# zama-ai/bounty-matrix-inversion

Hardware: AMD Instinct MI355X
Metric: PBS/sec per GPU + encrypted n x n inverse wall-clock (n=2,3,4) (higher is better)
Workload: dtype u64/f64

## Files before the change

bounty-matrix-inversion_amd/csrc/bmi_kernels_t64f.hip:

```cpp
#include <hip/hip_runtime.h>

#include "bmi_internal.hpp"
#include "fft_half_f64.hpp"
#include "fft_wave_f64.hpp"
#include "pair_sync.hpp"
#include "phase_prof.hpp"
#include "t64_common.hpp"
#include "t64_half_steps.hpp"

using t64::i64;
using t64::u64;
using namespace fftw;

namespace {

PH_ARRAY(g_phase_f)
using t64::f64_to_word;
using t64::mod_ab;
using t64::Scheme;
#ifndef BMI_T64F_CTS
#define BMI_T64F_CTS 4
#endif
constexpr int TF_CTS = BMI_T64F_CTS;
constexpr int TF_LDS_WORDS = TW_WORDS + 2 * TF_CTS * (SCRATCH_WORDS + N) + TF_CTS * BMI_AT_WORDS + 4 * TF_CTS;
static_assert(TF_LDS_WORDS <= BMI_LDS_WORDS_MAX, "TF_LDS_WORDS exceeds the 160 KB of LDS");
static_assert(SCRATCH_WORDS >= N, "a tile carries 512 complex partial sums to the partner");
static_assert(TF_CTS % 2 == 0, "both wavefronts of a pair must be in the same barrier group");

__global__ void __launch_bounds__(256) k_bsk_to_fft_t64(const u64 *__restrict__ std_polys, double *__restrict__ limb_polys,
                                                        const double *__restrict__ g_tw, uint32_t n_polys, int prec) {
    const int limbs = t64::limbs_of(prec);
    __shared__ double lds[TW_WORDS + 4 * SCRATCH_WORDS];
    for (int i = threadIdx.x; i < TW_WORDS; i += blockDim.x) lds[i] = g_tw[i];
    __syncthreads();
    const int wave = threadIdx.x >> 6, lane = threadIdx.x & 63;
    const uint32_t item = blockIdx.x * 4 + wave;
    if (item >= n_polys * (uint32_t)limbs) return;
    const uint32_t poly = item / limbs;
    const int j = (int)(item % limbs);
    double *scratch = lds + TW_WORDS + wave * SCRATCH_WORDS;
    double x[16];
    static_for<0, 16>([&](auto J) { x[J] = (double)t64::limb_of((i64)std_polys[(size_t)poly * N + lane + 64 * J], j, prec); });
    forward(x, lane, lds, scratch);
    double2 *dst = reinterpret_cast<double2 *>(limb_polys + (size_t)item * N);
    static_for<0, 8>([&](auto Cc) { dst[Cc * 64 + lane] = double2{x[Cc], x[Cc + 8]}; });
}

template <int L, int BG, bool STATS, bool GLWE>
__global__ void __launch_bounds__(128 * TF_CTS)
    k_blind_rotate_t64f(const u64 *__restrict__ small_cts, const uint32_t *__restrict__ lut_ids, const u64 *__restrict__ luts,
                        const double *__restrict__ bsk, const double *__restrict__ g_tw, u64 *__restrict__ out,
                        uint32_t count, uint32_t n, unsigned long long *__restrict__ stat) {
    constexpr int CTS = TF_CTS;
    constexpr int LIMBS = Scheme<48>::LIMBS, LB = Scheme<48>::BITS, PRE = Scheme<48>::PRE, AB = 64 - PRE;
    static_assert(2.0 * L * N * (double)(1ull << (BG - 1)) * (double)(1ull << (LB - 1)) <= 0x1p45, "limb sums must stay below 2^45");
    static_assert(LIMBS == 2 && L * BG < AB, "two limbs; the decomposed bits lie inside the key precision");
    extern __shared__ double lds[];
    double *tiles = lds + TW_WORDS;
    double *accs = tiles + 2 * CTS * SCRATCH_WORDS;
    double *at_base = accs + 2 * CTS * N;
    uint32_t *flags = reinterpret_cast<uint32_t *>(at_base + CTS * BMI_AT_WORDS);
    const int wave = threadIdx.x >> 6, lane = threadIdx.x & 63;
    const int ctl = wave >> 1, c = wave & 1;
    if (threadIdx.x < 4 * CTS) flags[threadIdx.x] = 0;
    for (int i = threadIdx.x; i < TW_WORDS; i += blockDim.x) lds[i] = g_tw[i];
    const uint32_t ct_raw = blockIdx.x * CTS + ctl;
    const bool live = ct_raw < count;
    const uint32_t ct = live ? ct_raw : count - 1;
    double *tile = tiles + wave * SCRATCH_WORDS;
    const double *ptile = tiles + (wave ^ 1) * SCRATCH_WORDS;
    double *accf = accs + wave * N;
    uint16_t *at = reinterpret_cast<uint16_t *>(at_base + ctl * BMI_AT_WORDS);
    uint32_t *f_pub = flags + wave, *f_pub_partner = flags + (wave ^ 1);
    uint32_t *f_ack = flags + 2 * CTS + wave, *f_ack_partner = flags + 2 * CTS + (wave ^ 1);
    const u64 *lwe = small_cts + (size_t)ct * (n + 1);
    t64::stage_lwe<LOG_N + 1>(at, lwe, n, lane + 64 * c, 128);
    __syncthreads();
    {
        const u64 *tv = luts + (size_t)(lut_ids[ct] & (BMI_LUT_CAP - 1)) * N;
        const uint32_t bt = at[n];
        static_for<0, 16>([&](auto J) {
            const uint32_t e = (lane + 64 * J + bt) & (2 * N - 1);
            const u64 v = tv[e & (N - 1)];
            const u64 w0 = c ? ((e & N) ? (u64)0 - v : v) : (u64)0;
            t64::set_acc<PRE>(accf[lane + 64 * J], w0);
        });
    }

    uint32_t hand = 0;
    double dev = 0.0;
    PH_DECL();
    double keep[16];
    static_for<0, 16>([&](auto J) { keep[J] = accf[lane + 64 * J]; });
    for (uint32_t i = 0; i < n; i++) {
        PH_MARK(7);
        barrier_if(threadIdx.x >= 64 * CTS);
        PH_MARK(0);
        const uint32_t a_t = at[i];
        const double *bsk_c = bsk + ((size_t)i * 4 * L + c * 2 * L) * LIMBS * N;
        __builtin_amdgcn_s_setprio(0);
        wave_sync();
        double r[16];
        {
            double vr[16], vs[16];
            static_for<0, 16>([&](auto J) {
                vr[J] = accf[((lane + 2 * N - a_t) + 64 * J) & (N - 1)];
                vs[J] = keep[J];
            });
            sched_fence();
            static_for<0, 16>([&](auto J) {
                const uint32_t e = ((lane + 2 * N - a_t) + 64 * J) & (2 * N - 1);
                const double d = mod_ab<AB>(((e & N) ? -vr[J] : vr[J]) - vs[J]);
                r[J] = t64::rounded_top_f64<L, BG, AB>(d);
            });
        }
        PH_MARK(1);
        double X[L][16];
        auto row_ptr = [&](int t) {
            const int j = t / (2 * L), q = t % (2 * L), lev = q % L, col = q < L ? (c ^ 1) : c;
            return reinterpret_cast<const double2 *>(bsk_c + ((size_t)(lev * 2 + col) * LIMBS + j) * N);
        };
        double2 kb[2][8];
        auto fetch = [&](double2 (&dst)[8], int t) { static_for<0, 8>([&](auto P) { dst[P] = row_ptr(t)[P * 64 + lane]; }); };
        ForwardTwiddles ftw;
        load_forward_twiddles(ftw, lane, lds);
        sched_fence();
        static_for<0, L>([&](auto LEV) {
            constexpr int lev = L - 1 - LEV;
            pin();
            static_for<0, 16>([&](auto J) {
                if constexpr (lev == 0) {
                    X[0][J] = r[J];
                } else {
                    const double rn = __builtin_floor(__builtin_fma(r[J], 1.0 / (double)(1ull << BG), 0.5));
                    X[lev][J] = __builtin_fma(-(double)(1ull << BG), rn, r[J]);
                    r[J] = rn;
                }
            });
            if constexpr (lev == 0) {
                fetch(kb[0], 0);
                pin();
            }
            forward(X[lev], lane, ftw, tile);
        });
        __builtin_amdgcn_s_setprio(1);
        PH_MARK(2);
        barrier_if(threadIdx.x < 64 * CTS);
        PH_MARK(0);
        double acc[16];
        static_for<0, LIMBS * 2 * L>([&](auto T) {
            constexpr int t = T, j = t / (2 * L), q = t % (2 * L), lev = q % L, cur = t & 1;
            if constexpr (q == 0) hand++;
            if constexpr (t + 1 < LIMBS * 2 * L && q != 2 * L - 1) fetch(kb[cur ^ 1], t + 1);
            sched_fence();
            static_for<0, 8>([&](auto P) {
                const double xr = X[lev][P], xi = X[lev][P + 8];
                if constexpr (lev == 0) {
                    acc[P] = __builtin_fma(xr, kb[cur][P].x, -(xi * kb[cur][P].y));
                    acc[P + 8] = __builtin_fma(xr, kb[cur][P].y, xi * kb[cur][P].x);
                } else {
                    acc[P] = __builtin_fma(xr, kb[cur][P].x, __builtin_fma(-xi, kb[cur][P].y, acc[P]));
                    acc[P + 8] = __builtin_fma(xr, kb[cur][P].y, __builtin_fma(xi, kb[cur][P].x, acc[P + 8]));
                }
            });
            if constexpr (q == L - 1) {
                wave_sync();
                static_for<0, 8>([&](auto P) {
                    reinterpret_cast<double2 *>(tile)[P * 64 + lane] = double2{acc[P], acc[P + 8]};
                });
                pair_post(f_pub, hand);
            }
            pin();
            if constexpr (q == 2 * L - 1) {
                PH_MARK(3);
                pair_wait(f_pub_partner, hand);
                PH_MARK(4);
                static_for<0, 8>([&](auto P) {
                    const double2 p = reinterpret_cast<const double2 *>(ptile)[P * 64 + lane];
                    acc[P] += p.x;
                    acc[P + 8] += p.y;
                });
                pin();
                pair_ack(f_ack, hand);
                pin();
                PH_MARK(5);
                inverse(acc, lane, lds, tile, [&]() {
                    pin();
                    pair_wait(f_ack_partner, hand);
                    pin();
                });
                PH_MARK(6);
                if constexpr (t + 1 < LIMBS * 2 * L) {
                    fetch(kb[cur ^ 1], t + 1);
                    pin();
                }
                static_for<0, 16>([&](auto J) {
                    double x = __builtin_rint(acc[J]);
                    if constexpr (STATS) dev = __builtin_fmax(dev, __builtin_fabs(acc[J] - x));
                    if constexpr (j > 0) {
                        constexpr double W = (double)(1ull << (AB - LB * j));
                        x = __builtin_fma(-W, __builtin_rint(x * (1.0 / W)), x);
                        keep[J] = mod_ab<AB>(__builtin_fma(x, (double)(1ull << (LB * j)), accf[lane + 64 * J]));
                        accf[lane + 64 * J] = keep[J];
                    } else {
                        accf[lane + 64 * J] += x;
                    }
                });
                pin();
            }
        });
    }

    PH_MARK(7);
    PH_STORE(g_phase_f, wave, lane);
    if constexpr (STATS) atomicMax(stat, (unsigned long long)__double_as_longlong(dev));
    if (!live) return;
    wave_sync();
    if constexpr (GLWE) {
        u64 *g = out + (size_t)ct * (2 * N) + c * N;
        static_for<0, 16>([&](auto J) { t64::store_glwe_word<PRE, AB>(g, accf, t64::ResidueSlot<N, 0>{}, lane + 64 * J); });
        return;
    }
    u64 *o = out + (size_t)ct * (N + 1);
    if (c == 0) {
        static_for<0, 16>([&](auto J) {
            const uint32_t m = lane + 64 * J;
            const u64 v = f64_to_word(accf[m]) << PRE;
            if (m == 0) o[0] = v;
            else o[N - m] = (u64)0 - v;
        });
    } else if (lane == 0) {
        o[N] = f64_to_word(accf[0]) << PRE;
    }
}

using namespace t64h;
constexpr int LF_LDS_WORDS = ffth::HT_WORDS + 2 * N + 2 * H_MAX_L * N + 2 * 2 * N + BMI_AT_WORDS;
static_assert(LF_LDS_WORDS <= BMI_LDS_WORDS_MAX, "LF_LDS_WORDS exceeds the 160 KB of LDS");

__global__ void __launch_bounds__(256) k_bsk_to_latf_t64(const u64 *__restrict__ std_polys, double *__restrict__ lat_polys,
                                                         const double *__restrict__ g_tw_h, uint32_t n_polys, int prec) {
    const int limbs = t64::limbs_of(prec);
    __shared__ double lds[ffth::HT_WORDS + 4 * H_HALF];
    for (int i = threadIdx.x; i < ffth::HT_WORDS; i += blockDim.x) lds[i] = g_tw_h[i];
    __syncthreads();
    const int wave = threadIdx.x >> 6, lane = threadIdx.x & 63;
    const int h = wave & 1;
    const uint32_t item = blockIdx.x * 2 + (wave >> 1);
    const bool ok = item < n_polys * (uint32_t)limbs;
    const uint32_t poly = ok ? item / limbs : 0;
    const int j = ok ? (int)(item % limbs) : 0;
    double2 *tile = reinterpret_cast<double2 *>(lds + ffth::HT_WORDS + wave * H_HALF);
    if (ok) {
        double re[4], im[4];
        static_for<0, 4>([&](auto R) {
            const uint32_t m = 2 * (lane + 64 * R) + h;
            re[R] = (double)t64::limb_of((i64)std_polys[(size_t)poly * N + m], j, prec);
            im[R] = (double)t64::limb_of((i64)std_polys[(size_t)poly * N + m + 512], j, prec);
        });
        ffth::C v[4];
        forward_half_of(h, re, im, v, lane, lds);
        static_for<0, 4>([&](auto R) { tile[R * 64 + lane] = double2{v[R].r, v[R].i}; });
    }
    __syncthreads();
    if (ok) {
        const double2 *te = reinterpret_cast<const double2 *>(lds + ffth::HT_WORDS + (wave & ~1) * H_HALF), *to = te + H_HALF / 2;
        double2 *o = reinterpret_cast<double2 *>(lat_polys + (size_t)item * N);
        static_for<0, 2>([&](auto Q2) {
            const int q = (h * 2 + Q2) * 64 + lane;
            const double2 e = te[q], od = to[q];
            o[2 * q] = double2{e.x + od.x, e.y + od.y};
            o[2 * q + 1] = double2{e.x - od.x, e.y - od.y};
        });
    }
}

template <int L, int BG, bool STATS, bool GLWE>
__global__ void __launch_bounds__(H_THREADS)
    k_blind_rotate_lat_t64f(const u64 *__restrict__ small_cts, const uint32_t *__restrict__ lut_ids, const u64 *__restrict__ luts,
                            const double *__restrict__ bsk_latf, const double *__restrict__ g_tw_h, u64 *__restrict__ out,
                            uint32_t count, uint32_t n, unsigned long long *__restrict__ stat) {
    constexpr int LIMBS = Scheme<48>::LIMBS, LB = Scheme<48>::BITS, PRE = Scheme<48>::PRE, AB = 64 - PRE;
    static_assert(2.0 * L * N * (double)(1ull << (BG - 1)) * (double)(1ull << (LB - 1)) <= 0x1p45, "limb sums must stay below 2^45");
    static_assert(LIMBS == 2 && L <= H_MAX_L && L * BG < AB, "two limbs, at most three levels");
    extern __shared__ double lds[];
    double *acc = lds + ffth::HT_WORDS;
    double2 *tiles = reinterpret_cast<double2 *>(lds + ffth::HT_WORDS + 2 * N);
    double2 *SD = tiles + H_MAX_L * N;
    uint16_t *at = reinterpret_cast<uint16_t *>(SD + 2 * N);
    const int tid = threadIdx.x, wave = tid >> 6, lane = tid & 63;
    for (int i = tid; i < ffth::HT_WORDS; i += H_THREADS) lds[i] = g_tw_h[i];
    const uint32_t ct = blockIdx.x;
    const u64 *lwe = small_cts + (size_t)ct * (n + 1);
    t64::stage_lwe<LOG_N + 1>(at, lwe, n, tid, H_THREADS);
    __syncthreads();
    {
        const u64 *tv = luts + (size_t)(lut_ids[ct] & (BMI_LUT_CAP - 1)) * N;
        const uint32_t bt = at[n];
        t64::load_test_poly<N, PRE>(acc, acc_slot, tv, bt, tid);
    }
    __syncthreads();
    const int mj = tid >> 9, mo = (tid >> 8) & 1, mq = tid & 255;
    uint32_t since_centred = 0;
    double dev = 0.0;

    for (uint32_t i = 0; i < n; i++) {
        const uint32_t a_t = at[i];
        if (a_t == 0) continue;
        const double *bi = bsk_latf + (size_t)i * 4 * L * LIMBS * N;
        double2 klo[2 * L], khi[2 * L];
        static_for<0, 2 * L>([&](auto R) {
            const double2 *row = reinterpret_cast<const double2 *>(bi + ((size_t)(R * 2 + mo) * LIMBS + mj) * N);
            klo[R] = row[2 * mq];
            khi[R] = row[2 * mq + 1];
        });
        if (wave < 4 * L) {
            const int c = wave / (2 * L), lev = (wave % (2 * L)) >> 1, h = wave & 1;
            const double *ac = acc + c * N;
            double x[8];
            double vr[8], vs[8];
            const uint32_t e0 = (2 * lane + h + 2 * N - a_t) & (2 * N - 1);
            const uint32_t t0 = e0 >> 1, pbase = (e0 & 1) * H_HALF;
            static_for<0, 8>([&](auto J) {
                const uint32_t t = t0 + 64 * (J & 3) + 256 * (J >> 2);
                vr[J] = ac[pbase + (t & (H_HALF - 1))];
                vs[J] = ac[h * H_HALF + lane + 64 * (J & 3) + 256 * (J >> 2)];
            });
            static_for<0, 8>([&](auto J) {
                const uint32_t t = t0 + 64 * (J & 3) + 256 * (J >> 2);
                const double dd = mod_ab<AB>(((t >> 9) & 1) ? -vr[J] - vs[J] : vr[J] - vs[J]);
                x[J] = t64::digit<L, BG, AB>(dd, lev);
            });
            const double re[4] = {x[0], x[1], x[2], x[3]}, im[4] = {x[4], x[5], x[6], x[7]};
            ffth::C v[4];
            forward_half_of(h, re, im, v, lane, lds);
            double2 *tile = tiles + (size_t)(wave >> 1) * H_HALF + h * (H_HALF / 2);
            static_for<0, 4>([&](auto R) { tile[R * 64 + lane] = double2{v[R].r, v[R].i}; });
        }
        __syncthreads();
        {
            ffth::C ylo{0.0, 0.0}, yhi{0.0, 0.0};
            static_for<0, 2 * L>([&](auto R) {
                const double2 e = tiles[(size_t)R * H_HALF + mq], od = tiles[(size_t)R * H_HALF + H_HALF / 2 + mq];
                mac_pair(ylo, yhi, e, od, klo[R], khi[R]);
            });
            const double2 w = reinterpret_cast<const double2 *>(lds + ffth::HT_W)[mq];
            sum_diff_store(SD + (size_t)(mj * 2 + mo) * H_HALF, mq, ylo, yhi, w);
        }
        __syncthreads();
        if (wave < 4 * LIMBS) {
            const int j = wave >> 2, o = (wave >> 1) & 1, h = wave & 1;
            const double2 *sd = SD + (size_t)(j * 2 + o) * H_HALF + h * (H_HALF / 2);
            ffth::C v[4];
            read_sums(v, sd, lane);
            double re[4], im[4];
            if (h) ffth::inverse_half<1>(v, re, im, lane, lds);
            else ffth::inverse_half<0>(v, re, im, lane, lds);
            double *ao = acc + o * N + h * H_HALF + lane;
            static_for<0, 4>([&](auto R) {
                atomicAdd(ao + 64 * R, t64::place_limb<AB, LB, STATS>(re[R], j, dev));
                atomicAdd(ao + 64 * R + 256, t64::place_limb<AB, LB, STATS>(im[R], j, dev));
            });
        }
        __syncthreads();
        if (++since_centred == H_RECENTRE) {
            since_centred = 0;
            recentre<AB, 2>(acc, tid);
            __syncthreads();
        }
    }
    if constexpr (STATS) atomicMax(stat, (unsigned long long)__double_as_longlong(dev));
    if constexpr (GLWE) t64::store_glwe<N, PRE, AB>(out + (size_t)ct * (2 * N), acc, acc_slot, tid);
    else t64::extract_sample<N, PRE, AB>(out + (size_t)ct * (N + 1), acc, acc_slot, tid);
}

}

PH_EXPORT(bmi_debug_phase_prof_t64f, g_phase_f)

namespace bmit {

bool shape_supported_fft(int prec, uint32_t levels, uint32_t base_log) {
    return prec == 48 && base_log == 10 && (levels == 3 || levels == 2);
}

int launch_bsk_to_fft(const u64 *std_polys, double *limb_polys, const double *g_tw_fft, uint32_t n_polys, int prec, hipStream_t s) {
    if (prec != 48) return (int)hipErrorInvalidValue;
    const uint32_t items = n_polys * (uint32_t)t64::limbs_of(prec);
    hipLaunchKernelGGL(k_bsk_to_fft_t64, dim3((items + 3) / 4), dim3(256), 0, s, std_polys, limb_polys, g_tw_fft, n_polys, prec);
    BMI_LAUNCH_CHECK();
    return 0;
}

int launch_bsk_to_latf(const u64 *std_polys, double *lat_polys, const double *g_tw_h, uint32_t n_polys, int prec, hipStream_t s) {
    if (prec != 48 && prec != 42) return (int)hipErrorInvalidValue;
    const uint32_t items = n_polys * (uint32_t)t64::limbs_of(prec);
    hipLaunchKernelGGL(k_bsk_to_latf_t64, dim3((items + 1) / 2), dim3(256), 0, s, std_polys, lat_polys, g_tw_h, n_polys, prec);
    BMI_LAUNCH_CHECK();
    return 0;
}

int launch_blind_rotate_lat_fft(const u64 *small_cts, const uint32_t *lut_ids, const u64 *luts, const double *bsk_fft,
                                const double *g_tw_fft, u64 *out, uint32_t count, uint32_t n, int prec, uint32_t levels,
                                uint32_t base_log, unsigned long long *stat, bool glwe, hipStream_t s) {
    if (count == 0) return 0;
    if (!shape_supported_fft(prec, levels, base_log)) return (int)hipErrorInvalidValue;
    return with_levels_stats_glwe(levels, stat != nullptr, glwe, [&](auto L, auto STATS, auto GLWE) {
        return launch_with_lds<k_blind_rotate_lat_t64f<L, 10, STATS, GLWE>>(dim3(count), dim3(H_THREADS), (size_t)LF_LDS_WORDS * sizeof(double), s,
                                                                             small_cts, lut_ids, luts, bsk_fft, g_tw_fft, out, count, n, stat);
    });
}

int launch_blind_rotate_fft(const u64 *small_cts, const uint32_t *lut_ids, const u64 *luts, const double *bsk_fft,
                            const double *g_tw_fft, u64 *out, uint32_t count, uint32_t n, int prec, uint32_t levels,
                            uint32_t base_log, unsigned long long *stat, bool glwe, hipStream_t s) {
    if (count == 0) return 0;
    if (!shape_supported_fft(prec, levels, base_log)) return (int)hipErrorInvalidValue;
    return with_levels_stats_glwe(levels, stat != nullptr, glwe, [&](auto L, auto STATS, auto GLWE) {
        return launch_with_lds<k_blind_rotate_t64f<L, 10, STATS, GLWE>>(dim3((count + TF_CTS - 1) / TF_CTS), dim3(128 * TF_CTS),
                                                                         (size_t)TF_LDS_WORDS * sizeof(double), s, small_cts, lut_ids, luts, bsk_fft,
                                                                         g_tw_fft, out, count, n, stat);
    });
}

}
```

bounty-matrix-inversion_amd/csrc/fft_wave_f64.hpp:

```cpp
#pragma once
#include <type_traits>

#include <hip/hip_runtime.h>

namespace fftw {

constexpr int LOG_N = 10;
constexpr int N = 1 << LOG_N;
constexpr int ROWC = 72;
constexpr int SCRATCH_WORDS = 8 * ROWC * 2;
constexpr int TW_T1 = 0;
constexpr int TW_T2 = 1024;
constexpr int TW_WORDS = 1024 + 128;

template <int I, int E, class F>
__device__ __forceinline__ void static_for(F &&f) {
    if constexpr (I < E) {
        f(std::integral_constant<int, I>{});
        static_for<I + 1, E>(f);
    }
}

__device__ __forceinline__ void wave_sync() {
    __builtin_amdgcn_fence(__ATOMIC_RELEASE, "wavefront");
    __builtin_amdgcn_wave_barrier();
    __builtin_amdgcn_fence(__ATOMIC_ACQUIRE, "wavefront");
}
__device__ __forceinline__ void sched_fence() { __builtin_amdgcn_sched_barrier(0); }

struct C {
    double r, i;
};
__device__ __forceinline__ C operator+(C a, C b) { return C{a.r + b.r, a.i + b.i}; }
__device__ __forceinline__ C operator-(C a, C b) { return C{a.r - b.r, a.i - b.i}; }
template <bool INV>
__device__ __forceinline__ C mul_i(C a) {
    if constexpr (INV) return C{a.i, -a.r};
    else return C{-a.i, a.r};
}
template <bool INV>
__device__ __forceinline__ C cmul(C a, double wr, double wi) {
    if constexpr (INV) return C{__builtin_fma(a.r, wr, a.i * wi), __builtin_fma(a.i, wr, -(a.r * wi))};
    else return C{__builtin_fma(a.r, wr, -(a.i * wi)), __builtin_fma(a.r, wi, a.i * wr)};
}
__device__ __forceinline__ C fma_h(C a, C b, double sh) { return C{__builtin_fma(sh, b.r, a.r), __builtin_fma(sh, b.i, a.i)}; }

__device__ constexpr double TWIST_C[8] = {1.0, 0.98078528040323043, 0.92387953251128674, 0.83146961230254524,
                                          0.70710678118654757, 0.55557023301960229, 0.38268343236508984, 0.19509032201612833};
__device__ constexpr double TWIST_S[8] = {0.0, 0.19509032201612825, 0.38268343236508978, 0.55557023301960218,
                                          0.70710678118654746, 0.83146961230254524, 0.92387953251128674, 0.98078528040323043};

template <bool INV>
__device__ __forceinline__ void dft8(C (&x)[8]) {
    constexpr double s = INV ? -1.0 : 1.0;
    constexpr double h = 0.70710678118654752440;
    const C a0 = x[0] + x[4], d0 = x[0] - x[4];
    const C a1 = x[1] + x[5], t1 = x[1] - x[5];
    const C a2 = x[2] + x[6], t2 = x[2] - x[6];
    const C a3 = x[3] + x[7], t3 = x[3] - x[7];
    const C d1 = C{t1.r - s * t1.i, t1.i + s * t1.r};
    const C d2 = mul_i<INV>(t2);
    const C d3 = C{-t3.r - s * t3.i, s * t3.r - t3.i};
    const C b0 = a0 + a2, b2 = a0 - a2;
    const C b1 = a1 + a3, b3 = mul_i<INV>(a1 - a3);
    const C e0 = d0 + d2, e2 = d0 - d2;
    const C e1 = d1 + d3, e3 = mul_i<INV>(d1 - d3);
    x[0] = b0 + b1;
    x[4] = b0 - b1;
    x[2] = b2 + b3;
    x[6] = b2 - b3;
    x[1] = fma_h(e0, e1, h);
    x[5] = fma_h(e0, e1, -h);
    x[3] = fma_h(e2, e3, h);
    x[7] = fma_h(e2, e3, -h);
}

struct NoHook {
    __device__ __forceinline__ void operator()() const {}
};

template <bool INV, class Pre, class Emit>
__device__ __forceinline__ void dft8_emit(C (&x)[8], Pre &&pre, Emit &&emit) {
    constexpr double s = INV ? -1.0 : 1.0;
    constexpr double h = 0.70710678118654752440;
    const C a0 = x[0] + x[4], d0 = x[0] - x[4];
    const C a1 = x[1] + x[5], t1 = x[1] - x[5];
    const C a2 = x[2] + x[6], t2 = x[2] - x[6];
    const C a3 = x[3] + x[7], t3 = x[3] - x[7];
    const C d1 = C{t1.r - s * t1.i, t1.i + s * t1.r};
    const C d2 = mul_i<INV>(t2);
    const C d3 = C{-t3.r - s * t3.i, s * t3.r - t3.i};
    const C b0 = a0 + a2, b2 = a0 - a2;
    const C b1 = a1 + a3, b3 = mul_i<INV>(a1 - a3);
    const C e0 = d0 + d2, e2 = d0 - d2;
    const C e1 = d1 + d3, e3 = mul_i<INV>(d1 - d3);
    pre();
    x[0] = b0 + b1;
    emit(std::integral_constant<int, 0>{});
    x[4] = b0 - b1;
    emit(std::integral_constant<int, 4>{});
    sched_fence();
    x[2] = b2 + b3;
    emit(std::integral_constant<int, 2>{});
    x[6] = b2 - b3;
    emit(std::integral_constant<int, 6>{});
    sched_fence();
    x[1] = fma_h(e0, e1, h);
    emit(std::integral_constant<int, 1>{});
    x[5] = fma_h(e0, e1, -h);
    emit(std::integral_constant<int, 5>{});
    sched_fence();
    x[3] = fma_h(e2, e3, h);
    emit(std::integral_constant<int, 3>{});
    x[7] = fma_h(e2, e3, -h);
    emit(std::integral_constant<int, 7>{});
    sched_fence();
}

__device__ __forceinline__ int ex1_row(int lane) { return (lane >> 3) * ROWC + (lane & 7); }
__device__ __forceinline__ int ex2_base(int lane) { return (lane >> 3) * ROWC; }

template <class Mid = NoHook>
__device__ __forceinline__ void forward(double (&x)[16], int lane, const double *tw, double *scratch, Mid mid = Mid()) {
    const double2 *tw2 = reinterpret_cast<const double2 *>(tw);
    double2 *sc = reinterpret_cast<double2 *>(scratch);
    double2 w[8];
    static_for<0, 8>([&](auto K) { w[K] = tw2[TW_T1 / 2 + K * 64 + lane]; });
    sched_fence();
    C v[8];
    v[0] = C{x[0], x[8]};
    static_for<1, 8>([&](auto R) { v[R] = cmul<false>(C{x[R], x[R + 8]}, TWIST_C[R], TWIST_S[R]); });
    dft8<false>(v);
    static_for<0, 8>([&](auto K) { v[K] = cmul<false>(v[K], w[K].x, w[K].y); });
    const int r1 = ex1_row(lane), a = lane & 7, base = ex2_base(lane);
    wave_sync();
    static_for<0, 8>([&](auto K) { sc[K * ROWC + lane] = double2{v[K].r, v[K].i}; });
    wave_sync();
    static_for<0, 8>([&](auto B) {
        const double2 t = sc[r1 + 8 * B];
        v[B] = C{t.x, t.y};
    });
    static_for<1, 8>([&](auto D) { w[D] = tw2[TW_T2 / 2 + D * 8 + a]; });
    mid();
    sched_fence();
    dft8<false>(v);
    static_for<1, 8>([&](auto D) { v[D] = cmul<false>(v[D], w[D].x, w[D].y); });
    wave_sync();
    static_for<0, 8>([&](auto D) { sc[base + D * 8 + ((a + D) & 7)] = double2{v[D].r, v[D].i}; });
    wave_sync();
    static_for<0, 8>([&](auto A) {
        const double2 t = sc[base + a * 8 + ((A + a) & 7)];
        v[A] = C{t.x, t.y};
    });
    dft8<false>(v);
    static_for<0, 8>([&](auto Cc) {
        x[Cc] = v[Cc].r;
        x[Cc + 8] = v[Cc].i;
    });
}

struct ForwardTwiddles {
    double2 t1[8], t2[8];
};
__device__ __forceinline__ void load_forward_twiddles(ForwardTwiddles &f, int lane, const double *tw) {
    const double2 *tw2 = reinterpret_cast<const double2 *>(tw);
    static_for<0, 8>([&](auto K) { f.t1[K] = tw2[TW_T1 / 2 + K * 64 + lane]; });
    static_for<1, 8>([&](auto D) { f.t2[D] = tw2[TW_T2 / 2 + D * 8 + (lane & 7)]; });
}
template <class Mid = NoHook>
__device__ __forceinline__ void forward(double (&x)[16], int lane, const ForwardTwiddles &f, double *scratch, Mid mid = Mid()) {
    double2 *sc = reinterpret_cast<double2 *>(scratch);
    C v[8];
    v[0] = C{x[0], x[8]};
    static_for<1, 8>([&](auto R) { v[R] = cmul<false>(C{x[R], x[R + 8]}, TWIST_C[R], TWIST_S[R]); });
    dft8<false>(v);
    static_for<0, 8>([&](auto K) { v[K] = cmul<false>(v[K], f.t1[K].x, f.t1[K].y); });
    const int r1 = ex1_row(lane), a = lane & 7, base = ex2_base(lane);
    wave_sync();
    static_for<0, 8>([&](auto K) { sc[K * ROWC + lane] = double2{v[K].r, v[K].i}; });
    wave_sync();
    static_for<0, 8>([&](auto B) {
        const double2 t = sc[r1 + 8 * B];
        v[B] = C{t.x, t.y};
    });
    mid();
    sched_fence();
    dft8<false>(v);
    static_for<1, 8>([&](auto D) { v[D] = cmul<false>(v[D], f.t2[D].x, f.t2[D].y); });
    wave_sync();
    static_for<0, 8>([&](auto D) { sc[base + D * 8 + ((a + D) & 7)] = double2{v[D].r, v[D].i}; });
    wave_sync();
    static_for<0, 8>([&](auto A) {
        const double2 t = sc[base + a * 8 + ((A + a) & 7)];
        v[A] = C{t.x, t.y};
    });
    dft8<false>(v);
    static_for<0, 8>([&](auto Cc) {
        x[Cc] = v[Cc].r;
        x[Cc + 8] = v[Cc].i;
    });
}

template <class Pre = NoHook>
__device__ __forceinline__ void inverse(double (&x)[16], int lane, const double *tw, double *scratch, Pre pre = Pre()) {
    const double2 *tw2 = reinterpret_cast<const double2 *>(tw);
    double2 *sc = reinterpret_cast<double2 *>(scratch);
    const int r1 = ex1_row(lane), a = lane & 7, base = ex2_base(lane);
    double2 w[8];
    static_for<1, 8>([&](auto D) { w[D] = tw2[TW_T2 / 2 + D * 8 + a]; });
    sched_fence();
    C v[8];
    static_for<0, 8>([&](auto Cc) { v[Cc] = C{x[Cc], x[Cc + 8]}; });
    dft8_emit<true>(
        v,
        [&]() {
            pre();
            wave_sync();
        },
        [&](auto A) { sc[base + a * 8 + ((A + a) & 7)] = double2{v[A].r, v[A].i}; });
    wave_sync();
    static_for<0, 8>([&](auto D) {
        const double2 t = sc[base + D * 8 + ((a + D) & 7)];
        v[D] = C{t.x, t.y};
    });
    static_for<1, 8>([&](auto D) { v[D] = cmul<true>(v[D], w[D].x, w[D].y); });
    static_for<0, 8>([&](auto K) { w[K] = tw2[TW_T1 / 2 + K * 64 + lane]; });
    sched_fence();
    dft8_emit<true>(v, [&]() { wave_sync(); }, [&](auto B) { sc[r1 + 8 * B] = double2{v[B].r, v[B].i}; });
    wave_sync();
    static_for<0, 8>([&](auto K) {
        const double2 t = sc[K * ROWC + lane];
        v[K] = C{t.x, t.y};
    });
    static_for<0, 8>([&](auto K) { v[K] = cmul<true>(v[K], w[K].x, w[K].y); });
    dft8<true>(v);
    x[0] = v[0].r * (1.0 / 512);
    x[8] = v[0].i * (1.0 / 512);
    static_for<1, 8>([&](auto R) {
        const C t = cmul<true>(v[R], TWIST_C[R] * (1.0 / 512), TWIST_S[R] * (1.0 / 512));
        x[R] = t.r;
        x[R + 8] = t.i;
    });
}

__host__ __device__ __forceinline__ int eval_offset(int lane, int c) { return (c * 64 + lane) * 2; }

}
```

Baseline: 129,700.

## Reorder limb accumulation to batch pair exchanges and preload inverse twiddles

Reorders the blind-rotate external product so both limbs' partner publishes and takes are interleaved with the MAC segments. Both inverse FFTs then run back-to-back after the exchange, and the limb results are merged in one accumulator update. It adds an InverseTwiddles struct loaded once into registers for both inverses, and pins the wave index and lane into scalar and vector registers. The aim is to cut pair-sync stalls and repeated LDS twiddle loads, at the cost of more live registers (a second accumulator plus the twiddles), which may lower occupancy or cause spills.

```diff
diff --git a/bounty-matrix-inversion_amd/csrc/bmi_kernels_t64f.hip b/bounty-matrix-inversion_amd/csrc/bmi_kernels_t64f.hip
--- a/bounty-matrix-inversion_amd/csrc/bmi_kernels_t64f.hip
+++ b/bounty-matrix-inversion_amd/csrc/bmi_kernels_t64f.hip
@@ -60,19 +60,15 @@
     double *accs = tiles + 2 * CTS * SCRATCH_WORDS;
     double *at_base = accs + 2 * CTS * N;
     uint32_t *flags = reinterpret_cast<uint32_t *>(at_base + CTS * BMI_AT_WORDS);
-    const int wave = threadIdx.x >> 6, lane = threadIdx.x & 63;
+    const int wave = __builtin_amdgcn_readfirstlane(threadIdx.x >> 6), lane = threadIdx.x & 63;
     const int ctl = wave >> 1, c = wave & 1;
     if (threadIdx.x < 4 * CTS) flags[threadIdx.x] = 0;
     for (int i = threadIdx.x; i < TW_WORDS; i += blockDim.x) lds[i] = g_tw[i];
     const uint32_t ct_raw = blockIdx.x * CTS + ctl;
     const bool live = ct_raw < count;
     const uint32_t ct = live ? ct_raw : count - 1;
-    double *tile = tiles + wave * SCRATCH_WORDS;
-    const double *ptile = tiles + (wave ^ 1) * SCRATCH_WORDS;
     double *accf = accs + wave * N;
     uint16_t *at = reinterpret_cast<uint16_t *>(at_base + ctl * BMI_AT_WORDS);
-    uint32_t *f_pub = flags + wave, *f_pub_partner = flags + (wave ^ 1);
-    uint32_t *f_ack = flags + 2 * CTS + wave, *f_ack_partner = flags + 2 * CTS + (wave ^ 1);
     const u64 *lwe = small_cts + (size_t)ct * (n + 1);
     t64::stage_lwe<LOG_N + 1>(at, lwe, n, lane + 64 * c, 128);
     __syncthreads();
@@ -93,10 +89,18 @@
     double keep[16];
     static_for<0, 16>([&](auto J) { keep[J] = accf[lane + 64 * J]; });
     for (uint32_t i = 0; i < n; i++) {
+        int wave_i = wave;
+        asm volatile("" : "+s"(wave_i));
         PH_MARK(7);
-        barrier_if(threadIdx.x >= 64 * CTS);
+        barrier_if(wave_i >= CTS);
         PH_MARK(0);
         const uint32_t a_t = at[i];
+        double *tile = tiles + wave_i * SCRATCH_WORDS;
+        const double *ptile = tiles + (wave_i ^ 1) * SCRATCH_WORDS;
+        uint32_t *f_pub = flags + wave_i, *f_pub_partner = flags + (wave_i ^ 1);
+        uint32_t *f_ack = flags + 2 * CTS + wave_i, *f_ack_partner = flags + 2 * CTS + (wave_i ^ 1);
+        int lane_a = lane;
+        asm volatile("" : "+v"(lane_a));
         const double *bsk_c = bsk + ((size_t)i * 4 * L + c * 2 * L) * LIMBS * N;
         __builtin_amdgcn_s_setprio(0);
         wave_sync();
@@ -104,12 +108,12 @@
         {
             double vr[16], vs[16];
             static_for<0, 16>([&](auto J) {
-                vr[J] = accf[((lane + 2 * N - a_t) + 64 * J) & (N - 1)];
+                vr[J] = accf[((lane_a + 2 * N - a_t) + 64 * J) & (N - 1)];
                 vs[J] = keep[J];
             });
             sched_fence();
             static_for<0, 16>([&](auto J) {
-                const uint32_t e = ((lane + 2 * N - a_t) + 64 * J) & (2 * N - 1);
+                const uint32_t e = ((lane_a + 2 * N - a_t) + 64 * J) & (2 * N - 1);
                 const double d = mod_ab<AB>(((e & N) ? -vr[J] : vr[J]) - vs[J]);
                 r[J] = t64::rounded_top_f64<L, BG, AB>(d);
             });
@@ -117,13 +121,13 @@
         PH_MARK(1);
         double X[L][16];
         auto row_ptr = [&](int t) {
-            const int j = t / (2 * L), q = t % (2 * L), lev = q % L, col = q < L ? (c ^ 1) : c;
+            const int seg = t / L, lev = t % L, j = seg >> 1, col = (seg & 1) ? c : (c ^ 1);
             return reinterpret_cast<const double2 *>(bsk_c + ((size_t)(lev * 2 + col) * LIMBS + j) * N);
         };
         double2 kb[2][8];
         auto fetch = [&](double2 (&dst)[8], int t) { static_for<0, 8>([&](auto P) { dst[P] = row_ptr(t)[P * 64 + lane]; }); };
         ForwardTwiddles ftw;
-        load_forward_twiddles(ftw, lane, lds);
+        load_forward_twiddles(ftw, lane_a, lds);
         sched_fence();
         static_for<0, L>([&](auto LEV) {
             constexpr int lev = L - 1 - LEV;
@@ -141,74 +145,94 @@
                 fetch(kb[0], 0);
                 pin();
             }
-            forward(X[lev], lane, ftw, tile);
+            forward(X[lev], lane_a, ftw, tile);
         });
         __builtin_amdgcn_s_setprio(1);
         PH_MARK(2);
-        barrier_if(threadIdx.x < 64 * CTS);
+        barrier_if(wave_i < CTS);
         PH_MARK(0);
-        double acc[16];
-        static_for<0, LIMBS * 2 * L>([&](auto T) {
-            constexpr int t = T, j = t / (2 * L), q = t % (2 * L), lev = q % L, cur = t & 1;
-            if constexpr (q == 0) hand++;
-            if constexpr (t + 1 < LIMBS * 2 * L && q != 2 * L - 1) fetch(kb[cur ^ 1], t + 1);
+        const uint32_t h0 = hand + 1, h1 = hand + 2;
+        hand = h1;
+        double acc[16], acc0[16];
+        auto publish = [&](uint32_t h) {
+            wave_sync();
+            static_for<0, 8>([&](auto P) {
+                reinterpret_cast<double2 *>(tile)[P * 64 + lane] = double2{acc[P], acc[P + 8]};
+            });
+            pair_post(f_pub, h);
+        };
+        auto take = [&](double (&a)[16], uint32_t h) {
+            PH_MARK(3);
+            pair_wait(f_pub_partner, h);
+            PH_MARK(4);
+            static_for<0, 8>([&](auto P) {
+                const double2 p = reinterpret_cast<const double2 *>(ptile)[P * 64 + lane];
+                a[P] += p.x;
+                a[P + 8] += p.y;
+            });
+            pin();
+            pair_ack(f_ack, h);
+            pin();
+            PH_MARK(5);
+        };
+        int lane_i = lane;
+        asm volatile("" : "+v"(lane_i));
+        InverseTwiddles itw;
+        static_for<0, 4 * L>([&](auto T) {
+            constexpr int t = T, seg = t / L, lev = t % L, cur = t & 1;
+            if constexpr (t + 1 < 4 * L) fetch(kb[cur ^ 1], t + 1);
             sched_fence();
+            double (&a)[16] = seg == 1 ? acc0 : acc;
             static_for<0, 8>([&](auto P) {
                 const double xr = X[lev][P], xi = X[lev][P + 8];
                 if constexpr (lev == 0) {
-                    acc[P] = __builtin_fma(xr, kb[cur][P].x, -(xi * kb[cur][P].y));
-                    acc[P + 8] = __builtin_fma(xr, kb[cur][P].y, xi * kb[cur][P].x);
+                    a[P] = __builtin_fma(xr, kb[cur][P].x, -(xi * kb[cur][P].y));
+                    a[P + 8] = __builtin_fma(xr, kb[cur][P].y, xi * kb[cur][P].x);
                 } else {
-                    acc[P] = __builtin_fma(xr, kb[cur][P].x, __builtin_fma(-xi, kb[cur][P].y, acc[P]));
-                    acc[P + 8] = __builtin_fma(xr, kb[cur][P].y, __builtin_fma(xi, kb[cur][P].x, acc[P + 8]));
+                    a[P] = __builtin_fma(xr, kb[cur][P].x, __builtin_fma(-xi, kb[cur][P].y, a[P]));
+                    a[P + 8] = __builtin_fma(xr, kb[cur][P].y, __builtin_fma(xi, kb[cur][P].x, a[P + 8]));
                 }
             });
-            if constexpr (q == L - 1) {
-                wave_sync();
-                static_for<0, 8>([&](auto P) {
-                    reinterpret_cast<double2 *>(tile)[P * 64 + lane] = double2{acc[P], acc[P + 8]};
-                });
-                pair_post(f_pub, hand);
+            if constexpr (lev == L - 1 && seg == 0) publish(h0);
+            if constexpr (lev == L - 1 && seg == 2) {
+                pin();
+                PH_MARK(3);
+                pair_wait(f_ack_partner, h0);
+                PH_MARK(4);
+                pin();
+                publish(h1);
             }
             pin();
-            if constexpr (q == 2 * L - 1) {
-                PH_MARK(3);
-                pair_wait(f_pub_partner, hand);
-                PH_MARK(4);
-                static_for<0, 8>([&](auto P) {
-                    const double2 p = reinterpret_cast<const double2 *>(ptile)[P * 64 + lane];
-                    acc[P] += p.x;
-                    acc[P + 8] += p.y;
-                });
-                pin();
-                pair_ack(f_ack, hand);
-                pin();
-                PH_MARK(5);
-                inverse(acc, lane, lds, tile, [&]() {
-                    pin();
-                    pair_wait(f_ack_partner, hand);
-                    pin();
-                });
-                PH_MARK(6);
-                if constexpr (t + 1 < LIMBS * 2 * L) {
-                    fetch(kb[cur ^ 1], t + 1);
-                    pin();
-                }
-                static_for<0, 16>([&](auto J) {
-                    double x = __builtin_rint(acc[J]);
-                    if constexpr (STATS) dev = __builtin_fmax(dev, __builtin_fabs(acc[J] - x));
-                    if constexpr (j > 0) {
-                        constexpr double W = (double)(1ull << (AB - LB * j));
-                        x = __builtin_fma(-W, __builtin_rint(x * (1.0 / W)), x);
-                        keep[J] = mod_ab<AB>(__builtin_fma(x, (double)(1ull << (LB * j)), accf[lane + 64 * J]));
-                        accf[lane + 64 * J] = keep[J];
-                    } else {
-                        accf[lane + 64 * J] += x;
-                    }
-                });
+            if constexpr (lev == L - 1 && seg == 1) take(acc0, h0);
+            if constexpr (lev == L - 1 && seg == 3) {
+                take(acc, h1);
+                load_inverse_twiddles(itw, lane_i, lds);
                 pin();
             }
         });
+        auto ack_hook = [&]() {
+            pin();
+            pair_wait(f_ack_partner, h1);
+            pin();
+        };
+        inverse(acc0, lane_i, itw, tile, ack_hook);
+        double x0[16];
+        static_for<0, 16>([&](auto J) {
+            x0[J] = __builtin_rint(acc0[J]);
+            if constexpr (STATS) dev = __builtin_fmax(dev, __builtin_fabs(acc0[J] - x0[J]));
+        });
+        pin();
+        inverse(acc, lane_i, itw, tile);
+        PH_MARK(6);
+        static_for<0, 16>([&](auto J) {
+            double x = __builtin_rint(acc[J]);
+            if constexpr (STATS) dev = __builtin_fmax(dev, __builtin_fabs(acc[J] - x));
+            constexpr double W = (double)(1ull << (AB - LB));
+            x = __builtin_fma(-W, __builtin_rint(x * (1.0 / W)), x);
+            keep[J] = mod_ab<AB>(__builtin_fma(x, (double)(1ull << LB), accf[lane_i + 64 * J] + x0[J]));
+            accf[lane_i + 64 * J] = keep[J];
+        });
+        pin();
     }
 
     PH_MARK(7);
diff --git a/bounty-matrix-inversion_amd/csrc/fft_wave_f64.hpp b/bounty-matrix-inversion_amd/csrc/fft_wave_f64.hpp
--- a/bounty-matrix-inversion_amd/csrc/fft_wave_f64.hpp
+++ b/bounty-matrix-inversion_amd/csrc/fft_wave_f64.hpp
@@ -243,6 +243,51 @@
     });
 }
 
+struct InverseTwiddles {
+    double2 t2[8], t1[8];
+};
+__device__ __forceinline__ void load_inverse_twiddles(InverseTwiddles &f, int lane, const double *tw) {
+    const double2 *tw2 = reinterpret_cast<const double2 *>(tw);
+    static_for<1, 8>([&](auto D) { f.t2[D] = tw2[TW_T2 / 2 + D * 8 + (lane & 7)]; });
+    static_for<0, 8>([&](auto K) { f.t1[K] = tw2[TW_T1 / 2 + K * 64 + lane]; });
+}
+template <class Pre = NoHook>
+__device__ __forceinline__ void inverse(double (&x)[16], int lane, const InverseTwiddles &f, double *scratch, Pre pre = Pre()) {
+    double2 *sc = reinterpret_cast<double2 *>(scratch);
+    const int r1 = ex1_row(lane), a = lane & 7, base = ex2_base(lane);
+    C v[8];
+    static_for<0, 8>([&](auto Cc) { v[Cc] = C{x[Cc], x[Cc + 8]}; });
+    dft8_emit<true>(
+        v,
+        [&]() {
+            pre();
+            wave_sync();
+        },
+        [&](auto A) { sc[base + a * 8 + ((A + a) & 7)] = double2{v[A].r, v[A].i}; });
+    wave_sync();
+    static_for<0, 8>([&](auto D) {
+        const double2 t = sc[base + D * 8 + ((a + D) & 7)];
+        v[D] = C{t.x, t.y};
+    });
+    static_for<1, 8>([&](auto D) { v[D] = cmul<true>(v[D], f.t2[D].x, f.t2[D].y); });
+    sched_fence();
+    dft8_emit<true>(v, [&]() { wave_sync(); }, [&](auto B) { sc[r1 + 8 * B] = double2{v[B].r, v[B].i}; });
+    wave_sync();
+    static_for<0, 8>([&](auto K) {
+        const double2 t = sc[K * ROWC + lane];
+        v[K] = C{t.x, t.y};
+    });
+    static_for<0, 8>([&](auto K) { v[K] = cmul<true>(v[K], f.t1[K].x, f.t1[K].y); });
+    dft8<true>(v);
+    x[0] = v[0].r * (1.0 / 512);
+    x[8] = v[0].i * (1.0 / 512);
+    static_for<1, 8>([&](auto R) {
+        const C t = cmul<true>(v[R], TWIST_C[R] * (1.0 / 512), TWIST_S[R] * (1.0 / 512));
+        x[R] = t.r;
+        x[R + 8] = t.i;
+    });
+}
+
 __host__ __device__ __forceinline__ int eval_offset(int lane, int c) { return (c * 64 + lane) * 2; }
 
 }
```

Result: faster. 133,300 (median of 6 runs) (+2.8%).
